# ipfs/go-libp2p-pubsub

Measured on AMD Instinct MI355X. Metric: deliveries/sec (peer×msg) at 1M peers, 1/2/4/8 GPU; % of HBM roofline, higher is better.
Workload: dtype u64

## Files before the change

### go-libp2p-pubsub_amd/csrc/api.cpp

```cpp
#include <algorithm>
#include <cstdio>
#include <cstdlib>
#include <cstring>

#include "engine.hpp"
#include "psengine_plan.h"

using namespace psamd;

namespace {

TopicHost* join_topic(ps_engine* e, uint32_t topic) {
  if (!topic_ok(e, topic)) {
    e->fail(PS_E_STATE, "no such topic");
    return nullptr;
  }
  TopicHost& T = e->topics[topic];
  if (T.kind != Kind::Join) {
    e->fail(PS_E_STATE, "topic topology was set explicitly");
    return nullptr;
  }
  return &T;
}

// ... 117 lines not shown
  d.timing = env_flag("PSAMD_DRAIN_TIMING", d.timing);
  if (!env_flag("PSAMD_AB", false)) return;
  d.slab_ids = std::max<uint64_t>(kDrainSegBits, env_u64("PSAMD_DRAIN_SLAB_IDS", 10, d.slab_ids));
  if (const char* v = std::getenv("PSAMD_DRAIN_EMIT")) d.staged = std::strcmp(v, "direct") != 0;
  if (const char* v = std::getenv("PSAMD_DRAIN_ASYNC_OUT")) d.mapped_out = std::strcmp(v, "mapped") == 0;
  if (const char* v = std::getenv("PSAMD_DRAIN_SHARED")) d.share = std::strcmp(v, "private") != 0;
  if (const char* v = std::getenv("PSAMD_LOAD_COUNT")) d.load_rows = std::strcmp(v, "rows") == 0;
  d.spread_wide = env_u32("PSAMD_SPREAD_WIDE", 0, 1 << 30, d.spread_wide);
  d.spread_track_levels = env_u32("PSAMD_SPREAD_TRACK_LEVELS", 0, kAny, d.spread_track_levels);
  s.twin = env_flag("PSAMD_TWIN", s.twin);
  s.expand_opts = env_flag("PSAMD_NARROW", true) ? 0u : kExpandNoNarrow;
  s.chain_words_lead = env_u32("PSAMD_CHAIN_WORDS_LEAD", 0, 1 << 20, s.chain_words_lead);
  s.upload_reuse = env_flag("PSAMD_UPLOAD_REUSE", s.upload_reuse);
  s.sig_windows = env_flag("PSAMD_SIG_WINDOWS", s.sig_windows);
  s.fuse_reduce = env_flag("PSAMD_FUSE_REDUCE", s.fuse_reduce);
  ps_plan_opts o = e->opts;
  o.gpu_build = env_flag("PSAMD_GPU_BUILD", o.gpu_build);
  o.flood = env_flag("PSAMD_FLOOD", o.flood);
  if (!env_flag("PSAMD_PULL_PAIR", true)) o.chain_max = o.chain_max_groups = 1;
  if (const char* v = std::getenv("PSAMD_XCHG_OVERLAP")) o.xchg_overlap = std::atoi(v) != 0;
  o.chain_max = env_u32("PSAMD_CHAIN", 1, kChainLevels, o.chain_max);
  o.chain_max_groups = env_u32("PSAMD_CHAIN", 1, kChainLevels, o.chain_max_groups);
  o.overlap = env_flag("PSAMD_OVERLAP", o.overlap);
  o.overlap_min_rounds = env_u32("PSAMD_OVERLAP_ROUNDS", 2, kAny, o.overlap_min_rounds);
  o.overlap_min_bytes = env_u64("PSAMD_OVERLAP_BYTES", 10, o.overlap_min_bytes);
  o.pad_words = env_u32("PSAMD_PAD_WORDS", 2, kAny, o.pad_words);
  o.chain_tail = env_flag("PSAMD_CHAIN_TAIL", o.chain_tail);
  if (const char* v = std::getenv("PSAMD_LAUNCH_BYTES"))
    o.launch_bytes = static_cast<uint64_t>(std::max(0.0, std::atof(v)));
  o.chain_words = env_u32("PSAMD_CHAIN_WORDS", 256, 1 << 20, o.chain_words);
// ... 446 lines not shown
      got.emplace_back((static_cast<uint64_t>(e->last_msgs[i].start) << 32) | i, e->last_first + i);
  }
  std::sort(got.begin(), got.end());
  *n_out = got.size();
  if (got.size() > cap) return e->fail(PS_E_RANGE, "output buffer too small");
  for (size_t k = 0; k < got.size(); ++k) msg_out[k] = got[k].second;
  return PS_OK;
}

int ps_overlapped_windows(ps_engine* e, uint64_t* count_out) {
  if (!e || !count_out) return PS_E_INVAL;
  *count_out = e->overlapped;
  return PS_OK;
}

int ps_seen_digest(ps_engine* e, uint64_t* digest_out) {
  if (!e || !digest_out) return PS_E_INVAL;
  if (!e->have_window) return e->fail(PS_E_NOTREADY, "no completed run");
  if (const int rj = twin_join(e)) return rj;
  HIP_TRY(hipMemsetAsync(e->d_digest.p, 0, 8, e->stream), "clear digest");
  const bool timed = e->drain.env.timing && e->drain.ev_t[0];
  if (timed) HIP_TRY(hipEventRecord(e->drain.ev_t[0], e->stream), "event");
  HIP_TRY(launch_digest(e->rows.seen.as<uint64_t>(), e->rows.gen.as<uint8_t>(), e->rows.gen_cur, e->d_node_peer.as<uint32_t>(),
                        e->d_node_topic.as<uint16_t>(),
                        e->last_slot->topics.as<TopicDev>(), e->last_slot->groups.as<GroupDev>(), e->n_nodes, e->d_digest.as<uint64_t>(), e->stream),
          "digest");
  if (timed) HIP_TRY(hipEventRecord(e->drain.ev_t[1], e->stream), "event");
  HIP_TRY(hipMemcpyAsync(digest_out, e->d_digest.p, 8, hipMemcpyDeviceToHost, e->stream), "read digest");
  HIP_TRY(hipStreamSynchronize(e->stream), "sync");
  if (timed) {
// ... 300 lines not shown
    case PS_PLAN_CHAIN: {
      const PairPlan& P = e->pair;
      if (index >= P.len.size() || P.len[index] < 3) {
        v = {0};
        break;
      }
      v = {P.len[index]};
      for (uint32_t k = P.lo[index]; k < P.hi[index]; ++k) {
        const ChainChunk& c = P.chain[k];
        v.insert(v.end(), {c.node_begin, c.node_end, c.topic, c.W, static_cast<uint64_t>(c.row0_hi) << 32 | c.row0_lo,
                           c.w0, c.S, c.levels, c.r0, c.group});
        for (uint32_t f = 0; f <= kChainLevels; ++f) v.push_back(c.first[f]);
      }
      break;
    }
    case PS_PLAN_SCHEDULE: {
      if (!L) return e->fail(PS_E_RANGE, "no window planned");
      const WindowSchedule& S = e->probe_sched;
      const size_t lv = L->level ? 1 : 0;
      v = {S.flood_rounds, S.pre_P, S.n_slots, S.reach_rows, S.mode, S.total, lv * S.lgrid.size(),
           lv * e->woff_host.size(), lv * e->desc_host.size(), S.seed_off.size()};
      if (lv) {
        v.insert(v.end(), S.lgrid.begin(), S.lgrid.end());
        v.insert(v.end(), e->woff_host.begin(), e->woff_host.end());
        v.insert(v.end(), e->desc_host.begin(), e->desc_host.end());
      }
      v.insert(v.end(), S.seed_off.begin(), S.seed_off.end());
      break;
    }
    default:
// ... 69 lines not shown
```

### go-libp2p-pubsub_amd/csrc/engine.hpp

```cpp
#pragma once
#include <hip/hip_runtime.h>

#include <array>
#include <chrono>
#include <cstdlib>
#include <cstdint>
#include <map>
#include <memory>
#include <string>
#include <utility>
#include <vector>

#include "dist.hpp"
#include "kernels.hpp"
#include "psengine.h"
#include "tree.hpp"

namespace psamd {

constexpr uint32_t kMaxRoundsCap = 4096;
constexpr uint32_t kAlignedRowsMax = 2 * (PS_MAX_ROUNDS + 1);
constexpr uint32_t kMaxStartRound = 200;
constexpr uint32_t kDefaultWindow = 65536;
constexpr uint32_t kMaxWindow = 1u << 30;
// ... 141 lines not shown
struct PullPlan {
  std::vector<uint64_t> key;
  uint64_t version = 0;
  std::vector<PullChunk> chunks;
  std::vector<uint32_t> off, gsplit;
  std::vector<uint64_t> bytes;
};
struct PairPlan {
  std::vector<uint64_t> key;
  uint64_t version = 0;
  std::vector<PullChunk> chunks;
  std::vector<ChainChunk> chain;
  std::vector<uint32_t> lo, hi, gsplit;
  std::vector<uint32_t> len;
  std::vector<uint8_t> kind;
};
struct FloodPlan {
  std::vector<uint64_t> key;
  uint64_t version = 0;
  std::vector<FloodTask> tasks;
  std::vector<FloodSeg> segs;
  std::vector<uint32_t> slot0, nslot;
  uint32_t slots = 1;
  uint32_t granules = 0;
};
struct GhostRound {
  std::vector<uint64_t> s_off, s_len, r_off, r_len;
  uint32_t pack0 = 0, pack1 = 0;
  uint64_t pack_units = 0;
  bool any = false;
// ... 42 lines not shown
  hipStream_t xstream = nullptr;
  hipEvent_t ev_run0 = nullptr, ev_run1 = nullptr;
  hipEvent_t ev_round = nullptr, ev_xchg = nullptr;
  ps_plan_opts opts = psamd::default_plan_opts();
  bool xchg_overlap = true;
  struct Switches {
    bool host_timing = false;
    bool flood_profile = false;
    std::string chain_prof_path;
    bool twin = true;
    bool sig_windows = true;
    bool fuse_reduce = true;
    bool upload_reuse = true;
    uint32_t expand_opts = 0;
    uint32_t chain_words_lead = 0;
  } env;
  std::vector<hipEvent_t> ev_k;
  uint32_t n_cus = 256, expand_grid = 2048;
  bool host_only = false;
  psamd::WindowLayout probe;
  psamd::WindowSchedule probe_sched;
  struct UploadShadow {
    uint64_t gen = 0;
    std::vector<uint8_t> data;
  };
  std::map<const psamd::DevBuf*, UploadShadow> upload_shadow;
  bool defer_into_signalled = false;
  uint64_t sig_seq = 0;
  struct PendingReduce {
    bool valid = false;
// ... 41 lines not shown
  bool graph_dirty = true, flags_dirty = true;
  uint64_t graph_epoch = 0, flags_epoch = 0;

  std::vector<uint32_t> woff_host, desc_host;
  psamd::DevBuf d_reach;
  std::vector<psamd::ReachPiece> reach_host;
  std::vector<uint64_t> reach_key;
  uint32_t n_reach = 0, reach_a = 0;
  psamd::PullPlan pull;
  psamd::DevBuf d_pull;
  uint64_t pull_up = ~0ull;
  psamd::DevBuf d_chain;
  std::vector<uint64_t> chain_fail_key;
  psamd::DevBuf d_chain_ovf;
  psamd::DevBuf d_chain_meta, d_chain_cnt, d_chain_scan;
  static constexpr uint64_t kNtBytes = 64ull << 20;
  psamd::PairPlan pair;
  psamd::DevBuf d_pp;
  uint64_t pair_up = ~0ull;
  std::vector<uint8_t> round_kind;

  uint32_t n_nodes = 0, n_pad = 16;
  std::vector<uint32_t> node_peer, row_ptr, col;
  std::vector<uint32_t> node_parent;
  std::vector<uint16_t> node_topic;
  std::vector<uint8_t> node_flags;

  psamd::DevBuf d_row_ptr, d_col, d_node_topic, d_node_flags, d_node_peer, d_node_parent;
  psamd::DevBuf d_ext0, d_ext1;
  struct RowSet {
// ... 368 lines not shown
    uint64_t epoch = ~0ull;
    std::vector<uint32_t> gslot;
    std::vector<uint32_t> plist;
    std::vector<std::vector<uint32_t>> pl_off;
    psamd::DevBuf d_gslot, d_plist;
  } dist_slots;

  struct Staging {
    uint8_t* h = nullptr;
    uint8_t* d = nullptr;
    size_t cap = 0;
  };
  struct RunSlot {
    Staging stg;
    psamd::DevBuf topics, woff, groups, partials, seeds;
    hipEvent_t ev_gate = nullptr;
    ps_stats st{};
    bool deferred = false;
    uint32_t r = 0, launches = 0;
    uint32_t mode = PS_MODE_COMPACT, flood_rounds = 0;
    hipEvent_t ev0 = nullptr, ev1 = nullptr;
    uint64_t* hs = nullptr;
    uint64_t* hs_dev = nullptr;
    uint64_t* ha = nullptr;
    uint64_t* sig = nullptr;
    uint64_t* sig_dev = nullptr;
    uint64_t seq = 0;
    bool signalled = false;
    uint32_t planned0 = 0;
    uint32_t true_rounds = 0;
// ... 119 lines not shown
```

### go-libp2p-pubsub_amd/csrc/kernels.hpp

```cpp
#pragma once
#include <hip/hip_runtime.h>

#include <cstdint>

namespace psamd {

enum : uint8_t {
  kNodeLive = 1,
  kNodeInternal = 2,
  kNodeSplit = 4,
};

constexpr uint32_t kRemoteBit = 0x80000000u;
constexpr uint32_t kRemoteRankShift = 27;
constexpr uint32_t kRemoteIdMask = (1u << kRemoteRankShift) - 1u;
constexpr int kMaxRanks = 16;

struct XItem {
  uint32_t node;
  uint32_t word;
  uint64_t mask;
};
constexpr uint32_t kRegionHeader = 16;

// ... 165 lines not shown
  uint32_t first[kChainLevels + 1];
  uint32_t lo[kChainLevels], hi[kChainLevels];
  uint32_t nbase, root;
};
static_assert(sizeof(ChainChunk) == 128, "two chunk descriptors per 256-B line");
hipError_t launch_chain_ranges(ChainChunk* chunks, uint32_t n, const uint32_t* row_ptr, uint32_t cap,
                               uint32_t* overflow, hipStream_t s);
hipError_t launch_chain_meta(ChainChunk* chunks, uint32_t n, const uint32_t* node_parent, const uint8_t* node_flags,
                             uint32_t* counts, void* scan_temp, size_t scan_bytes, uint32_t* meta, bool fill,
                             hipStream_t s);
size_t chain_meta_scan_bytes(uint32_t n);
hipError_t launch_pull_chain(const PullArgs& a, const ChainChunk* chunks, uint32_t n_chunks, uint32_t round,
                             bool record, bool nt, bool slices, bool inner_nt, uint32_t waves_per_cu,
                             hipStream_t s);
hipError_t launch_chain_parents(ChainChunk* chunks, uint32_t n, const uint32_t* node_parent, hipStream_t s);
constexpr uint32_t kPullSlots = 256;
constexpr uint32_t kPairSlots = kPullSlots;

struct FloodTask {
  uint32_t nb, ne;
  uint32_t topic, round;
  uint32_t slot0, nslot;
  uint32_t g_own, gsz;
  uint32_t p_lo, p_hi;
  uint32_t pg_lo, pg_hi;
  uint32_t pnode0, pgsz;
  uint32_t pseg;
  uint32_t seg;
};
struct FloodSeg {
// ... 727 lines not shown
```

### go-libp2p-pubsub_amd/csrc/plan.cpp

```cpp
#include <algorithm>
#include <cstring>

#include "engine.hpp"

namespace psamd {

uint64_t phys_word(const TopicDev& d, const std::vector<StartGroup>& G, uint64_t u, uint32_t w) {
  if (!(d.flags & kTopicGroups)) return d.wbase + u * d.W + w;
  for (const StartGroup& g : G)
    if (w < g.w0 + g.wn) return d.wbase + static_cast<uint64_t>(d.n_nodes) * g.w0 + u * g.wn + (w - g.w0);
  return d.wbase;
}

namespace {

uint32_t block_w(const TopicDev& d, const StartGroup& g) { return (d.flags & kTopicGroups) ? g.wn : d.W; }
uint64_t block_row0(const TopicDev& d, const StartGroup& g) {
  return d.wbase + ((d.flags & kTopicGroups) ? static_cast<uint64_t>(d.n_nodes) * g.w0 : 0);
}

}

int plan_window_layout(ps_engine* e, const std::vector<RunMsg>& msgs, const std::vector<WinSlice>& win,
                       WindowLayout& L) {
// ... 343 lines not shown
      if (!can(q, len)) continue;
      const double c = wb + rd[q] + (wb > 0 ? kLaunchBytes : 0.0) + best[q + len];
      if (c < best[q]) {
        best[q] = c;
        take[q] = static_cast<uint8_t>(len);
      }
    }
  }
  auto& C = PP.chunks;
  C.clear();
  PP.chain.clear();
  PP.lo.assign(rounds + 2, 0);
  PP.hi.assign(rounds + 2, 0);
  PP.gsplit.assign(rounds + 2, 0);
  PP.len.assign(rounds + 2, 0);
  const bool gpu = e->gpu_graph;
  std::vector<PullChunk> ghost;
  for (uint32_t q = first + 1; q <= rounds; ++q) {
    const uint32_t len = take[q];
    if (len == 1) {
      kind[q] = e->pull.bytes[q] ? PS_K_PULL : PS_K_NONE;
      continue;
    }
    PP.len[q] = len;
    if (len >= 3) {
      kind[q] = PS_K_CHAIN;
      for (uint32_t k = 1; k < len; ++k) kind[q + k] = PS_K_CHAIN2;
      PP.lo[q] = static_cast<uint32_t>(PP.chain.size());
      std::vector<ChainChunk> sliced;
      chain_parts(q, len, [&](uint32_t t, uint32_t gi, uint32_t d, uint32_t r0, uint32_t levels) {
// ... 17 lines not shown
            c.w0 = w0;
            c.S = std::min(z.S, W - w0);
            c.levels = static_cast<uint8_t>(levels);
            c.r0 = static_cast<uint8_t>(r0);
            c.group = static_cast<uint16_t>(gi);
            c.nbase = T.nbase;
            c.root = T.root_local ? T.nbase : kNoneNode;
            for (uint32_t k = 0; k <= levels && k <= kChainLevels; ++k)
              c.first[k] = T.nbase + (d + k < T.level_off.size() ? T.level_off[d + k] : T.n_nodes);
            (z.S < W ? sliced : PP.chain).push_back(c);
          }
      });
      PP.gsplit[q] = static_cast<uint32_t>(PP.chain.size());
      PP.chain.insert(PP.chain.end(), sliced.begin(), sliced.end());
      PP.hi[q] = static_cast<uint32_t>(PP.chain.size());
      q += len - 1;
      continue;
    }
    kind[q] = PS_K_PAIR;
    kind[q + 1] = PS_K_PAIR2;
    PP.lo[q] = static_cast<uint32_t>(C.size());
    ghost.clear();
    for (uint32_t t = 0; t < nt; ++t) {
      const TopicHost& T = e->topics[t];
      if (tab[t].W == 0) continue;
      for (uint32_t gi = 0; gi < L.groups[t].size(); ++gi) {
        const StartGroup& g = L.groups[t][gi];
        const uint32_t W = block_w(tab[t], g);
        uint32_t d, per;
        bool late = false;
// ... 570 lines not shown
```

### go-libp2p-pubsub_amd/csrc/run.cpp

```cpp
#include <algorithm>
#include <chrono>
#include <atomic>
#include <cstdio>
#include <cstdlib>
#include <cstring>
#include <iterator>
#include <thread>

#include "engine.hpp"
#include "gbuild.hpp"

namespace {
inline void cpu_relax() {
#if defined(__x86_64__) || defined(__i386__)
  __builtin_ia32_pause();
#else
  std::this_thread::yield();
#endif
}
}

namespace psamd {

namespace {
// ... 53 lines not shown
    uint32_t back[2] = {0, 0};
    HIP_TRY(hipMemcpyAsync(&back[0], e->d_chain_ovf.p, 4, hipMemcpyDeviceToHost, e->stream), "read chain overflow");
    HIP_TRY(hipMemcpyAsync(&back[1], e->d_chain_cnt.as<uint32_t>() + nk + 1 + nk, 4, hipMemcpyDeviceToHost,
                           e->stream),
            "read chain entries");
    HIP_TRY(hipStreamSynchronize(e->stream), "sync");
    if (back[0]) {
      *overflow = true;
      return PS_OK;
    }
    HIP_TRY(e->d_chain_meta.ensure(std::max<size_t>(back[1], 1) * 4), "alloc chain entries");
    HIP_TRY(launch_chain_meta(e->d_chain.as<ChainChunk>(), nk, e->d_node_parent.as<uint32_t>(),
                              e->d_node_flags.as<uint8_t>(), e->d_chain_cnt.as<uint32_t>(), nullptr, 0,
                              e->d_chain_meta.as<uint32_t>(), true, e->stream),
            "chain entries");
  }
  e->pair_up = e->pair.version;
  return PS_OK;
}

int upload_flood(ps_engine* e) {
  if (e->flood.version == e->flood_up) return PS_OK;
  const auto& TK = e->flood.tasks;
  const auto& SG = e->flood.segs;
  const size_t n = TK.size();
  HIP_TRY(e->d_flood_tasks.ensure(std::max<size_t>(n, 1) * sizeof(FloodTask)), "alloc flood tasks");
  HIP_TRY(e->d_flood_segs.ensure(std::max<size_t>(SG.size(), 1) * sizeof(FloodSeg)), "alloc flood segments");
  bool fresh = false;
  HIP_TRY(e->d_flood_gran.ensure(std::max<size_t>(e->flood.granules, 1) * 8, &fresh), "alloc flood granules");
  if (fresh) HIP_TRY(hipMemsetAsync(e->d_flood_gran.p, 0, e->d_flood_gran.bytes, e->stream), "clear granules");
// ... 198 lines not shown
  uint32_t reach_a = 0;
  bool twin = false, pcap = false, alt_sets = false, overlap = false, fold = false, sigwin = false;
  std::vector<uint64_t> gkey;
  WindowStart ws{};
  const void* staged[4] = {nullptr, nullptr, nullptr, nullptr};
  ExpandArgs a{};
  PullArgs pa{};
  uint64_t* arr[2] = {nullptr, nullptr};
  uint64_t* partials = nullptr;
  uint64_t* stats = nullptr;
  uint32_t stats_rows = 0, n_waves = 0;
  bool upfront = false;
  bool zero_copy = false;
  std::vector<const uint8_t*> peer_region;
  bool gate_done = false, reach_a_done = false;
  bool cprof = false;
  bool host_stats_written = false;
  bool reduce_side = false;
  size_t ev_used = 0;
  std::vector<uint32_t> ev_round;
  uint32_t launches = 0;
  uint32_t r = 0;
  std::vector<uint64_t> s_off, s_len, r_off, r_len;
  Clock::time_point t_w0, t_w1, t_w3, t_first, t_enq;

  bool defers(uint32_t r) {
    return e->defer_last && e->defer_into && !record && !timed && r <= PS_MAX_ROUNDS &&
           (e->world == 1 || L.planned0 <= PS_MAX_ROUNDS);
  }

// ... 450 lines not shown
  }

  int launch_chain(uint32_t r, bool xr) {
    const uint32_t len = e->pair.len[r];
    const uint32_t last = r + len - 1;
    const bool ntc =
        last == L.planned0 || (last < e->pull.bytes.size() && e->pull.bytes[last] >= ps_engine::kNtBytes);
    pa.slot_mod = kPairSlots;
    pa.row_ptr = e->d_row_ptr.as<uint32_t>();
    for (uint32_t k = 0; k < kChainLevels; ++k)
      pa.partials_r[k] = k < len ? partials + static_cast<size_t>(e->woff_host[r + k]) * kNumCtr : nullptr;
    HIP_TRY(time_mark(true), "event");
    ++launches;
    uint64_t* const prof = cprof ? e->d_chain_prof.as<uint64_t>() : nullptr;
    pa.prof = prof ? prof + static_cast<size_t>(e->pair.lo[r]) * kChainProf : nullptr;
    HIP_TRY(launch_pull_chain(pa, e->d_chain.as<ChainChunk>() + e->pair.lo[r], e->pair.gsplit[r] - e->pair.lo[r], r,
                              record, ntc, false, e->opts.chain_nt, e->opts.chain_waves, s),
            "pull chain");
    pa.prof = prof ? prof + static_cast<size_t>(e->pair.gsplit[r]) * kChainProf : nullptr;
    HIP_TRY(launch_pull_chain(pa, e->d_chain.as<ChainChunk>() + e->pair.gsplit[r], e->pair.hi[r] - e->pair.gsplit[r],
                              r, record, ntc, true, e->opts.chain_nt, e->opts.chain_waves, s),
            "pull chain (column slices)");
    pa.prof = nullptr;
    HIP_TRY(time_mark(false), "event");
    if (xr) HIP_TRY(hipStreamWaitEvent(s, e->ev_xchg, 0), "exchange join");
    return PS_OK;
  }

  int launch_pull_round(uint32_t r, bool pair, bool xr, hipStream_t xs) {
    const uint32_t rw = pair ? r + 1 : r;
    const bool nt = rw < e->pull.bytes.size() && (e->pull.bytes[rw] >= ps_engine::kNtBytes || rw == L.planned0);
    pa.partials = partials + static_cast<size_t>(e->woff_host[r]) * kNumCtr;
    pa.slot_mod = pair ? kPairSlots : kPullSlots;
// ... 781 lines not shown
```

### go-libp2p-pubsub_amd/psengine/__init__.py

```python
from __future__ import annotations

import ctypes as C
import os

import numpy as np

from . import _build

NONE = 0xFFFFFFFF
HOP_NONE = 0xFF
MAX_ROUNDS = 256

PS_OK = 0
ERRORS = {
    -1: "PS_E_INVAL", -2: "PS_E_NOMEM", -3: "PS_E_STATE", -4: "PS_E_NOPARENT",
    -5: "PS_E_UNREACHABLE", -6: "PS_E_DEVICE", -7: "PS_E_RANGE", -8: "PS_E_NOTREADY",
}
PART_PEER = 0
PART_SUBTREE = 1
F_RECORD_HOPS = 0x1
F_TIME_KERNELS = 0x2
F_NO_LAZY_SEEN = 0x4
F_COMPACT = 0x8
MODE_COMPACT, MODE_LEVEL_PULL, MODE_FLOOD = 0, 2, 3
# ... 162 lines not shown
    ("ps_blame_track", C.c_int, [_P, _u32p, C.c_size_t, C.c_size_t]),
    ("ps_blame_take", C.c_int, [_P, C.POINTER(_u64p), C.POINTER(_u32p), C.POINTER(_u32p), C.POINTER(_u32p),
                                C.POINTER(_u32p), C.POINTER(_u32p), _u64p, _u64p, _u64p, _u64p]),
    ("ps_peer_report", C.c_int, [_P, _u32p, C.c_size_t, C.c_uint32, C.POINTER(Report), C.c_size_t]),
    ("ps_report_track", C.c_int, [_P, _u32p, C.c_size_t, C.c_uint32]),
    ("ps_report_take", C.c_int, [_P, C.POINTER(Report), C.c_size_t, _u64p, _u64p]),
    ("ps_dist_report", C.c_int, [_P, _u32p, C.c_size_t, C.c_uint32, C.POINTER(Report), C.c_size_t]),
    ("ps_dist_cut", C.c_int, [_P, _u32p, C.c_size_t, _u64p, _u64p, _u64p, _u64p]),
    ("ps_dist_blame", C.c_int, [_P, _u32p, C.c_size_t, C.POINTER(_u64p), C.POINTER(_u32p), C.POINTER(_u32p),
                                C.POINTER(_u32p), C.POINTER(_u32p), C.POINTER(_u32p), _u64p]),
    ("ps_topic_spread", C.c_int, [_P, _u32p, C.c_size_t, _u64p, _u64p, _u64p, _u64p, _u64p, _u64p]),
    ("ps_spread_track", C.c_int, [_P, _u32p, C.c_size_t]),
    ("ps_spread_take", C.c_int, [_P, _u64p, _u64p, _u64p, _u64p, _u64p, _u64p, _u64p, _u64p]),
    ("ps_seen_digest", C.c_int, [_P, _u64p]),
    ("ps_overlapped_windows", C.c_int, [_P, _u64p]),
    ("ps_msg_encode", C.c_int, [C.POINTER(MessageC), C.c_char_p, C.c_size_t, C.POINTER(C.c_size_t)]),
    ("ps_msg_decode", C.c_int, [C.c_char_p, C.c_size_t, C.POINTER(MessageBuf), C.POINTER(C.c_size_t)]),
    ("ps_dist_unique_id", C.c_int, [C.POINTER(C.c_uint8)]),
    ("ps_dist_init", C.c_int, [_P, C.POINTER(DistConfig), C.POINTER(C.c_uint8)]),
    ("ps_device_count", C.c_int, [_i32p]),
    ("ps_dist_ipc_id", C.c_int, [C.POINTER(C.c_uint8)]),
    ("ps_dist_init_ipc", C.c_int, [_P, C.POINTER(DistConfig), C.POINTER(C.c_uint8)]),
    ("ps_loopback_create", C.c_int, [C.c_int32, C.POINTER(_P)]),
    ("ps_loopback_destroy", None, [_P]),
    ("ps_dist_init_loopback", C.c_int, [_P, C.POINTER(DistConfig), _P]),
    ("ps_partition_owner", C.c_int, [_u32, _u32, _u32p, _u32, C.POINTER(DistConfig), _i32p]),
]

G_NODE_PEER, G_NODE_PARENT, G_NODE_TOPIC, G_NODE_FLAGS, G_ROW_PTR, G_COL, G_TOPIC, G_BUILD = range(8)
NODE_LIVE, NODE_INTERNAL, NODE_SPLIT = 1, 2, 4
# ... 669 lines not shown
        from . import plan

        return graph_get(plan.lib(), self._h, what, index)

    def graph_topic(self, topic: int) -> dict:
        return graph_topic(self.graph(G_TOPIC, topic))

    def build_report(self) -> dict:
        return build_report(self.graph(G_BUILD))

    def overlapped_windows(self) -> int:
        d = C.c_uint64()
        self._check(self._L.ps_overlapped_windows(self._h, C.byref(d)))
        return d.value

    def dist_init(self, rank: int, world: int, unique_id: bytes, partition: int = PART_PEER,
                  split_depth: int = 0):
        dc = DistConfig(rank, world, partition, split_depth)
        uid = (C.c_uint8 * 128).from_buffer_copy(unique_id)
        self._check(self._L.ps_dist_init(self._h, C.byref(dc), uid))

    def dist_init_ipc(self, rank: int, world: int, group_id: bytes, partition: int = PART_PEER,
                      split_depth: int = 0, copy: bool = False, inplace: bool = False):
        flags = (DIST_F_COPY if copy else 0) | (DIST_F_INPLACE if inplace else 0)
        dc = DistConfig(rank, world, partition, split_depth, flags, 0)
        gid = (C.c_uint8 * 128).from_buffer_copy(group_id)
        self._check(self._L.ps_dist_init_ipc(self._h, C.byref(dc), gid))

    def dist_init_loopback(self, group: "Loopback", rank: int, partition: int = PART_PEER,
                           split_depth: int = 0, copy: bool = False, inplace: bool = False):
# ... 69 lines not shown
```

### go-libp2p-pubsub_amd/psengine/_build.py

```python
from __future__ import annotations

import os
import subprocess

PKG = os.path.dirname(os.path.dirname(os.path.abspath(__file__)))
REPO = os.path.dirname(PKG)
CSRC = os.path.join(PKG, "csrc")
LIBDIR = os.path.join(PKG, "lib")
LIB = os.path.join(LIBDIR, "libpsengine.so")
HIPCC = os.environ.get("HIPCC", "/opt/rocm/bin/hipcc")
ARCH = "gfx950"

SOURCES = ["kernels.hip", "pull.hip", "flood.hip", "gbuild.hip", "drain.hip", "graph.cpp", "plan.cpp", "run.cpp", "api.cpp",
           "drain_tables.cpp", "drain_standing.cpp", "drain.cpp", "drain_shared.cpp", "drain_sink.cpp", "drain_topics.cpp",
           "drain_load.cpp", "drain_hops.cpp", "drain_downstream.cpp", "drain_cut.cpp", "drain_report.cpp",
           "drain_dist.cpp", "drain_spread.cpp", "drain_blame.cpp", "drain_blame_track.cpp", "drain_spread_track.cpp",
           "tree.cpp", "dist.cpp", "codec.cpp", "pubsub.cpp"]
HEADERS = ["kernels.hpp", "devutil.hpp", "gbuild.hpp", "tree.hpp", "dist.hpp", "engine.hpp", "drain_impl.hpp"]


def _stale() -> bool:
    if not os.path.exists(LIB):
        return True
    t = os.path.getmtime(LIB)
    deps = [os.path.join(CSRC, f) for f in SOURCES + HEADERS]
    deps.append(os.path.join(REPO, "include", "psengine.h"))
    deps.append(os.path.join(REPO, "include", "pubsub.hpp"))
    deps.append(os.path.join(REPO, "include", "psengine_plan.h"))
# ... 56 lines not shown
```

### go-libp2p-pubsub_amd/psengine/plan.py

```python
from __future__ import annotations

import ctypes as C

import numpy as np

from . import (DistConfig, EngineError, G_BUILD, G_TOPIC, PART_PEER, PlanOpts, _P, _p, _u32arr, build_report,
               graph_get, graph_topic, load)

(INFO, NODES, PARENT, GHOST_REF, TOPIC, LAYOUT, ROUND_KIND, PULL, PAIR, XCHG, SEGS, SHIP, PACK, CHAIN,
 SCHEDULE) = range(15)
CHAIN_FIELDS = ("node_begin", "node_end", "topic", "W", "row0", "w0", "S", "levels", "r0", "group")
CHAIN_LEVELS = 6
CHUNK_FIELDS = ("node_begin", "node_end", "topic", "W", "row0", "e_lo", "e_hi", "gin", "gout", "group",
                "p_lo", "p_hi", "c_lo")
PROTOTYPES = [
    ("ps_plan_create", C.c_int, [C.c_uint32, C.c_uint32, C.POINTER(C.c_uint32), C.POINTER(C.c_uint32),
                                 C.POINTER(DistConfig), C.POINTER(_P)]),
    ("ps_plan_destroy", None, [_P]),
    ("ps_plan_set_msg_window", C.c_int, [_P, C.c_uint32]),
    ("ps_plan_window", C.c_int, [_P, C.POINTER(C.c_uint32), C.POINTER(C.c_uint32), C.c_size_t, C.c_uint32]),
    ("ps_plan_get", C.c_int, [_P, C.c_uint32, C.c_uint32, C.POINTER(C.c_uint64), C.c_size_t,
                              C.POINTER(C.c_size_t)]),
    ("ps_graph_get", C.c_int, [_P, C.c_uint32, C.c_uint32, C.POINTER(C.c_uint64), C.c_size_t,
                               C.POINTER(C.c_size_t)]),
]
# ... 142 lines not shown
        out["desc"] = out["desc"].reshape(-1, 3)
        return out

    def chain(self, q: int):
        v = self.get(CHAIN, q)
        n = int(v[0])
        if n == 0:
            return 0, []
        body = v[1:].reshape(-1, len(CHAIN_FIELDS) + CHAIN_LEVELS + 1)
        out = []
        for row in body:
            c = dict(zip(CHAIN_FIELDS, (int(x) for x in row[:len(CHAIN_FIELDS)])))
            c["first"] = [int(x) for x in row[len(CHAIN_FIELDS):]]
            out.append(c)
        return n, out
```

### include/psengine.h

```cpp
#ifndef PSENGINE_H
#define PSENGINE_H

#include <stddef.h>
#include <stdint.h>

#ifdef __cplusplus
extern "C" {
#endif

#define PS_NONE 0xFFFFFFFFu
#define PS_HOP_NONE 0xFFu
#define PS_MAX_ROUNDS 256

enum ps_status {
  PS_OK = 0,
  PS_E_INVAL = -1,
  PS_E_NOMEM = -2,
  PS_E_STATE = -3,
  PS_E_NOPARENT = -4,
  PS_E_UNREACHABLE = -5,
  PS_E_DEVICE = -6,
  PS_E_RANGE = -7,
  PS_E_NOTREADY = -8
};
// ... 264 lines not shown

int ps_topic_spread(ps_engine* e, const uint32_t* topic, size_t n,
                    uint64_t* reached_out, uint64_t* deliv_out,
                    uint64_t* unreached_out, uint64_t* stranded_out,
                    uint64_t* copies_out, uint64_t* dup_out);
int ps_spread_track(ps_engine* e, const uint32_t* topic, size_t n);
int ps_spread_take(ps_engine* e,
                   uint64_t* reached_out, uint64_t* deliv_out,
                   uint64_t* unreached_out, uint64_t* stranded_out,
                   uint64_t* copies_out, uint64_t* dup_out,
                   uint64_t* n_windows_out, uint64_t* n_truncated_out);
int ps_seen_digest(ps_engine* e, uint64_t* digest_out);

int ps_overlapped_windows(ps_engine* e, uint64_t* count_out);

#define PS_PART_PEER 0u
#define PS_PART_SUBTREE 1u
#define PS_UNIQUE_ID_BYTES 128

typedef struct ps_dist_config {
  int32_t rank;
  int32_t world;
  uint32_t partition;
  uint32_t split_depth;
  uint32_t flags;
  uint32_t reserved;
} ps_dist_config;
#define PS_DIST_F_COPY 0x1u
#define PS_DIST_F_INPLACE 0x2u

// ... 52 lines not shown
```

### include/psengine_plan.h

```cpp
#ifndef PSENGINE_PLAN_H
#define PSENGINE_PLAN_H

#include "psengine.h"

#ifdef __cplusplus
extern "C" {
#endif

int ps_plan_create(uint32_t n_peers, uint32_t n_topics, const uint32_t* roots, const uint32_t* parents,
                   const ps_dist_config* dc, ps_engine** out);
void ps_plan_destroy(ps_engine* e);
int ps_plan_set_msg_window(ps_engine* e, uint32_t msg_window);
int ps_plan_window(ps_engine* e, const uint32_t* topic_of_msg, const uint32_t* start_round, size_t n_msgs,
                   uint32_t flags);

#define PS_PLAN_INFO 0
#define PS_PLAN_NODES 1
#define PS_PLAN_PARENT 2
#define PS_PLAN_GHOST_REF 3
#define PS_PLAN_TOPIC 4
#define PS_PLAN_LAYOUT 5
#define PS_PLAN_ROUND_KIND 6
#define PS_PLAN_PULL 7
#define PS_PLAN_PAIR 8
#define PS_PLAN_XCHG 9
#define PS_PLAN_SEGS 10
#define PS_PLAN_SHIP 11
#define PS_PLAN_PACK 12
#define PS_PLAN_CHAIN 13
#define PS_PLAN_SCHEDULE 14
int ps_plan_get(ps_engine* e, uint32_t what, uint32_t index, uint64_t* out, size_t cap, size_t* n_out);

#define PS_GRAPH_NODE_PEER 0
#define PS_GRAPH_NODE_PARENT 1
#define PS_GRAPH_NODE_TOPIC 2
#define PS_GRAPH_NODE_FLAGS 3
#define PS_GRAPH_ROW_PTR 4
#define PS_GRAPH_COL 5
#define PS_GRAPH_TOPIC 6
#define PS_GRAPH_BUILD 7
int ps_graph_get(ps_engine* e, uint32_t what, uint32_t index, uint64_t* out, size_t cap, size_t* n_out);

#ifdef __cplusplus
}
#endif
// ... 2 lines not shown
```

Baseline: 40030 billion.

## Replace chain pull with split reach and row-fill kernels for single-GPU windows

```diff
diff --git a/go-libp2p-pubsub_amd/csrc/api.cpp b/go-libp2p-pubsub_amd/csrc/api.cpp
--- a/go-libp2p-pubsub_amd/csrc/api.cpp
+++ b/go-libp2p-pubsub_amd/csrc/api.cpp
@@ -155,6 +155,11 @@
   s.upload_reuse = env_flag("PSAMD_UPLOAD_REUSE", s.upload_reuse);
   s.sig_windows = env_flag("PSAMD_SIG_WINDOWS", s.sig_windows);
   s.fuse_reduce = env_flag("PSAMD_FUSE_REDUCE", s.fuse_reduce);
+  s.chain_fill = env_flag("PSAMD_CHAIN_FILL", s.chain_fill);
+  s.chain_fill_bytes = env_u64("PSAMD_CHAIN_FILL_BYTES", 10, s.chain_fill_bytes);
+  s.chain_fill_row_words = env_u64("PSAMD_CHAIN_FILL_ROW_WORDS", 10, s.chain_fill_row_words);
+  s.chain_fill_waves = env_u32("PSAMD_CHAIN_FILL_WAVES", 0, 32, s.chain_fill_waves);
+  s.chain_fill_piece = env_u32("PSAMD_CHAIN_FILL_PIECE", 16, 1 << 16, s.chain_fill_piece);
   ps_plan_opts o = e->opts;
   o.gpu_build = env_flag("PSAMD_GPU_BUILD", o.gpu_build);
   o.flood = env_flag("PSAMD_FLOOD", o.flood);
@@ -631,6 +636,12 @@
   return PS_OK;
 }
 
+int ps_chain_fill_launches(ps_engine* e, uint64_t* count_out) {
+  if (!e || !count_out) return PS_E_INVAL;
+  *count_out = e->chain_fills;
+  return PS_OK;
+}
+
 int ps_seen_digest(ps_engine* e, uint64_t* digest_out) {
   if (!e || !digest_out) return PS_E_INVAL;
   if (!e->have_window) return e->fail(PS_E_NOTREADY, "no completed run");
@@ -961,6 +972,27 @@
       }
       break;
     }
+    case PS_PLAN_FILL: {
+      const PairPlan& P = e->pair;
+      if (index >= P.fill_hi.size() || P.fill_hi[index] <= P.fill_lo[index]) {
+        v = {0};
+        break;
+      }
+      v = {P.fill_hi[index] - P.fill_lo[index], P.fill_np[index], P.fill_blocks[index]};
+      for (uint32_t k = P.fill_lo[index]; k < P.fill_hi[index]; ++k) {
+        const FillSeg& f = P.fill[k];
+        v.insert(v.end(), {f.topic, f.W, f.row0, f.nbase, f.levels, f.piece0, f.blk0, f.pw});
+        for (uint32_t i = 0; i <= kChainLevels; ++i) v.push_back(f.first[i]);
+      }
+      for (uint32_t k = P.fill_lo[index]; k < P.fill_hi[index]; ++k) {
+        const FillSeg& f = P.fill[k];
+        for (uint32_t j = 0, n = fill_seg_pieces(f); j < n; ++j) {
+          const FillPiece p = fill_piece(f, j);
+          v.insert(v.end(), {p.w0, p.nw, p.node0, p.off0});
+        }
+      }
+      break;
+    }
     case PS_PLAN_SCHEDULE: {
       if (!L) return e->fail(PS_E_RANGE, "no window planned");
       const WindowSchedule& S = e->probe_sched;
diff --git a/go-libp2p-pubsub_amd/csrc/engine.hpp b/go-libp2p-pubsub_amd/csrc/engine.hpp
--- a/go-libp2p-pubsub_amd/csrc/engine.hpp
+++ b/go-libp2p-pubsub_amd/csrc/engine.hpp
@@ -179,6 +179,8 @@
   std::vector<uint32_t> lo, hi, gsplit;
   std::vector<uint32_t> len;
   std::vector<uint8_t> kind;
+  std::vector<FillSeg> fill;
+  std::vector<uint32_t> fill_lo, fill_hi, fill_blocks, fill_p0, fill_np;
 };
 struct FloodPlan {
   std::vector<uint64_t> key;
@@ -251,6 +253,11 @@
     bool upload_reuse = true;
     uint32_t expand_opts = 0;
     uint32_t chain_words_lead = 0;
+    bool chain_fill = true;
+    uint32_t chain_fill_piece = psamd::kFillPieceWords;
+    uint64_t chain_fill_bytes = 512ull << 20;
+    uint64_t chain_fill_row_words = psamd::kFillMinRowWords;
+    uint32_t chain_fill_waves = psamd::kFillWaves;
   } env;
   std::vector<hipEvent_t> ev_k;
   uint32_t n_cus = 256, expand_grid = 2048;
@@ -322,6 +329,8 @@
   std::vector<uint64_t> chain_fail_key;
   psamd::DevBuf d_chain_ovf;
   psamd::DevBuf d_chain_meta, d_chain_cnt, d_chain_scan;
+  psamd::DevBuf d_fill_segs, d_fill_pieces;
+  uint64_t chain_fills = 0;
   static constexpr uint64_t kNtBytes = 64ull << 20;
   psamd::PairPlan pair;
   psamd::DevBuf d_pp;
@@ -720,6 +729,7 @@
   struct RunSlot {
     Staging stg;
     psamd::DevBuf topics, woff, groups, partials, seeds;
+    psamd::DevBuf fill_pop;
     hipEvent_t ev_gate = nullptr;
     ps_stats st{};
     bool deferred = false;
diff --git a/go-libp2p-pubsub_amd/csrc/fill.hip b/go-libp2p-pubsub_amd/csrc/fill.hip
--- /dev/null
+++ b/go-libp2p-pubsub_amd/csrc/fill.hip
@@ -0,0 +1,219 @@
+#include <cstddef>
+
+#include "devutil.hpp"
+#include "kernels.hpp"
+
+namespace psamd {
+
+namespace {
+
+using namespace dev;
+
+typedef unsigned int u32x4 __attribute__((ext_vector_type(4)));
+
+__global__ __launch_bounds__(kBlock) void k_fill_pieces(const FillSeg* __restrict__ segs, uint32_t n_segs,
+                                                        FillPiece* __restrict__ pieces, uint32_t n_pieces) {
+  const uint32_t i = blockIdx.x * kBlock + threadIdx.x;
+  if (i >= n_pieces) return;
+  uint32_t lo = 0, hi = n_segs;
+  while (hi - lo > 1) {
+    const uint32_t mid = (lo + hi) >> 1;
+    if (segs[mid].piece0 <= i)
+      lo = mid;
+    else
+      hi = mid;
+  }
+  pieces[i] = fill_piece(segs[lo], i - segs[lo].piece0);
+}
+
+__global__ __launch_bounds__(64) void k_fill_popc(const FillSeg* __restrict__ segs, uint32_t n_segs,
+                                                  const uint64_t* __restrict__ a_cur, uint32_t* __restrict__ pop) {
+  const uint32_t si = blockIdx.x;
+  if (si >= n_segs) return;
+  const uint64_t* row = a_cur + segs[si].row0;
+  const uint32_t W = segs[si].W;
+  uint32_t n = 0;
+  for (uint32_t i = threadIdx.x; i < W; i += 64) n += static_cast<uint32_t>(__popcll(row[i]));
+  n = __reduce_add_sync(~0ull, n);
+  if (threadIdx.x == 0) pop[segs[si].topic] = n;
+}
+
+__device__ __forceinline__ uint64_t* fill_slots(const FillReachArgs& a, uint32_t i) {
+  switch (i) {
+    case 0: return a.partials_r[0];
+    case 1: return a.partials_r[1];
+    case 2: return a.partials_r[2];
+    case 3: return a.partials_r[3];
+    case 4: return a.partials_r[4];
+    default: return a.partials_r[5];
+  }
+}
+
+__global__ __launch_bounds__(kFillReachBlock) void k_fill_reach(FillReachArgs a) {
+  const uint32_t b = blockIdx.x;
+  uint32_t lo = 0, hi = a.n_segs;
+  while (hi - lo > 1) {
+    const uint32_t mid = (lo + hi) >> 1;
+    if (a.segs[mid].blk0 <= b)
+      lo = mid;
+    else
+      hi = mid;
+  }
+  const FillSeg* const S = a.segs + lo;
+  const uint32_t levels = S->levels, W = S->W, cur = a.gen_cur & 0xFF;
+  const uint32_t u0 = S->first[0], end = S->first[levels];
+  const uint32_t u = u0 + (b - S->blk0) * kFillReachBlock + threadIdx.x;
+  const bool in = u < end;
+  const uint32_t uc = in ? u : u0;
+  uint32_t k = 0;
+  for (uint32_t j = 1; j < kChainLevels; ++j) k += (j < levels && uc >= S->first[j]) ? 1u : 0u;
+  const uint32_t par = a.node_parent[uc];
+  const uint32_t par_prev = a.node_parent[uc - 1];
+  const bool live = a.node_flags[uc] & kNodeLive;
+  uint32_t p = par;
+  bool live_above = true;
+  for (uint32_t j = 0; j < k; ++j) {
+    live_above = live_above && (a.node_flags[p] & kNodeLive);
+    p = a.node_parent[p];
+  }
+  const bool up = in && live_above && a.gen[p] == cur;
+  const bool ok = up && live;
+  const bool first = up && par != par_prev;
+  if (ok) a.gen[uc] = static_cast<uint8_t>(cur);
+  const uint32_t lane = threadIdx.x & 63u, wave = threadIdx.x >> 6;
+  const uint64_t slot = (static_cast<uint64_t>(b) * (kFillReachBlock / 64) + wave) % a.slot_mod;
+  const uint64_t pop = a.pop[S->topic];
+  for (uint32_t j = 0; j < levels; ++j) {
+    const uint64_t nodes = __ballot(in && k == j);
+    if (nodes == 0) continue;
+    const uint64_t reached = __popcll(__ballot(ok && k == j));
+    const uint64_t parents = __popcll(__ballot(first && k == j));
+    const uint64_t pwords = (j == 0 && b == S->blk0 && wave == 0) ? W : 0u;
+    const uint64_t v7[7] = {reached * pop, reached * W, static_cast<uint64_t>(__popcll(nodes)), reached, parents,
+                            pwords, 0ull};
+    uint64_t* const partials = fill_slots(a, j);
+    if (partials && lane < kNumCtr) {
+      const uint64_t v = pull_ctr_pick(v7, lane);
+      if (v) atomicAdd(reinterpret_cast<unsigned long long*>(partials + slot * kNumCtr + lane),
+                       static_cast<unsigned long long>(v));
+    }
+  }
+}
+
+template <bool kNT>
+__device__ __forceinline__ void fill_store16(uint64_t* p, const u32x4& v) {
+  if constexpr (kNT)
+    __builtin_nontemporal_store(v, reinterpret_cast<u32x4*>(p));
+  else
+    *reinterpret_cast<u32x4*>(p) = v;
+}
+
+template <bool kNT>
+__global__ __launch_bounds__(64) void k_fill_rows(const FillPiece* __restrict__ pieces, uint32_t n_pieces,
+                                                  const uint64_t* __restrict__ a_cur, uint64_t* __restrict__ seen,
+                                                  const uint8_t* __restrict__ gen, uint32_t gen_cur) {
+  constexpr uint32_t kU = 8;
+  constexpr uint32_t kGenWords = (kFillPieceNodes + 2 + 3) / 4 + 2;
+  __shared__ __attribute__((aligned(16))) uint64_t row[kChainWords];
+  __shared__ uint32_t genl[kGenWords];
+  if (blockIdx.x >= n_pieces) return;
+  const FillPiece* const pc = pieces + blockIdx.x;
+  const uint32_t lane = threadIdx.x;
+  const uint32_t cur = gen_cur & 0xFF;
+  const uint64_t w0 = pc->w0;
+  const uint32_t nw = pc->nw, W = pc->W, node0 = pc->node0, off0 = pc->off0;
+  const uint64_t* const src = a_cur + pc->row0;
+  const uint32_t nn = (off0 + nw + W - 1) / W;
+  const uint32_t g0 = node0 & ~3u;
+  const uint32_t nd = (((node0 + nn + 3u) & ~3u) - g0) >> 2;
+  const uint32_t* const gen32 = reinterpret_cast<const uint32_t*>(gen + g0);
+  for (uint32_t i = lane; i < nd; i += 64) genl[i] = gen32[i];
+  for (uint32_t i = lane; i < W; i += 64) row[i] = src[i];
+  __syncthreads();
+  const uint8_t* const genb = reinterpret_cast<const uint8_t*>(genl) + (node0 - g0);
+  const float rw = 1.0f / static_cast<float>(W);
+  auto split = [&](uint32_t i, int32_t& kk, int32_t& r) {
+    const uint32_t li = off0 + i;
+    kk = static_cast<int32_t>(static_cast<float>(li) * rw);
+    r = static_cast<int32_t>(li) - kk * static_cast<int32_t>(W);
+    const int32_t lo = r < 0, hi = r >= static_cast<int32_t>(W);
+    kk += hi - lo;
+    r += (lo - hi) * static_cast<int32_t>(W);
+  };
+  auto word = [&](uint32_t i) {
+    int32_t kk, r;
+    split(i, kk, r);
+    return genb[kk] == cur ? row[r] : 0ull;
+  };
+  uint64_t* const out = seen + w0;
+  const uint32_t h = static_cast<uint32_t>(w0 & 1u);
+  const uint32_t nu = (nw - h) >> 1;
+  if (h && lane == 0) out[0] = word(0);
+  if (((nw - h) & 1u) && lane == 1) out[nw - 1] = word(nw - 1);
+  const bool even = !(W & 1u) && !((off0 + h) & 1u);
+  for (uint32_t c0 = 0; c0 < nu; c0 += kU * 64) {
+    u32x4 x[kU];
+#pragma unroll
+    for (uint32_t q = 0; q < kU; ++q) {
+      const uint32_t c = min(c0 + q * 64 + lane, nu - 1);
+      int32_t kk, r;
+      split(h + 2 * c, kk, r);
+      if (even) {
+        x[q] = genb[kk] == cur ? *reinterpret_cast<const u32x4*>(row + r) : u32x4{0, 0, 0, 0};
+      } else {
+        const uint64_t a0 = genb[kk] == cur ? row[r] : 0ull;
+        const bool wrap = static_cast<uint32_t>(r) + 1 == W;
+        const uint64_t a1 = genb[kk + (wrap ? 1 : 0)] == cur ? row[wrap ? 0 : r + 1] : 0ull;
+        x[q] = u32x4{static_cast<uint32_t>(a0), static_cast<uint32_t>(a0 >> 32), static_cast<uint32_t>(a1),
+                     static_cast<uint32_t>(a1 >> 32)};
+      }
+    }
+#pragma unroll
+    for (uint32_t q = 0; q < kU; ++q) {
+      const uint32_t c = c0 + q * 64 + lane;
+      if (c < nu) fill_store16<kNT>(out + h + 2 * c, x[q]);
+    }
+  }
+}
+
+}
+
+hipError_t launch_fill_pieces(const FillSeg* segs, uint32_t n_segs, FillPiece* pieces, uint32_t n_pieces,
+                              hipStream_t s) {
+  if (n_segs == 0 || n_pieces == 0) return hipSuccess;
+  hipLaunchKernelGGL(k_fill_pieces, dim3((n_pieces + kBlock - 1) / kBlock), dim3(kBlock), 0, s, segs, n_segs, pieces,
+                     n_pieces);
+  return hipGetLastError();
+}
+
+hipError_t launch_fill_popc(const FillSeg* segs, uint32_t n_segs, const uint64_t* a_cur, uint32_t* pop, hipStream_t s) {
+  if (n_segs == 0) return hipSuccess;
+  hipLaunchKernelGGL(k_fill_popc, dim3(n_segs), dim3(64), 0, s, segs, n_segs, a_cur, pop);
+  return hipGetLastError();
+}
+
+hipError_t launch_fill_reach(const FillReachArgs& a, uint32_t n_blocks, hipStream_t s) {
+  if (a.n_segs == 0 || n_blocks == 0) return hipSuccess;
+  hipLaunchKernelGGL(k_fill_reach, dim3(n_blocks), dim3(kFillReachBlock), 0, s, a);
+  return hipGetLastError();
+}
+
+hipError_t launch_fill_rows(const FillPiece* pieces, uint32_t n_pieces, const uint64_t* a_cur, uint64_t* seen,
+                            const uint8_t* gen, uint32_t gen_cur, uint32_t waves_per_cu, hipStream_t s) {
+  if (n_pieces == 0) return hipSuccess;
+  static const size_t fixed = [] {
+    hipFuncAttributes fa{};
+    return hipFuncGetAttributes(&fa, reinterpret_cast<const void*>(k_fill_rows<false>)) == hipSuccess
+               ? fa.sharedSizeBytes
+               : size_t{0};
+  }();
+  size_t pad = 0;
+  if (waves_per_cu) {
+    const size_t per = (160u * 1024u) / waves_per_cu - 512u;
+    pad = per > fixed ? per - fixed : 0;
+  }
+  hipLaunchKernelGGL(k_fill_rows<false>, dim3(n_pieces), dim3(64), pad, s, pieces, n_pieces, a_cur, seen, gen, gen_cur);
+  return hipGetLastError();
+}
+
+}
diff --git a/go-libp2p-pubsub_amd/csrc/kernels.hpp b/go-libp2p-pubsub_amd/csrc/kernels.hpp
--- a/go-libp2p-pubsub_amd/csrc/kernels.hpp
+++ b/go-libp2p-pubsub_amd/csrc/kernels.hpp
@@ -203,6 +203,77 @@
                              bool record, bool nt, bool slices, bool inner_nt, uint32_t waves_per_cu,
                              hipStream_t s);
 hipError_t launch_chain_parents(ChainChunk* chunks, uint32_t n, const uint32_t* node_parent, hipStream_t s);
+struct FillSeg {
+  uint64_t row0;
+  uint32_t topic, W;
+  uint32_t nbase, levels;
+  uint32_t first[kChainLevels + 1];
+  uint32_t piece0;
+  uint32_t blk0;
+  uint32_t pw;
+};
+static_assert(sizeof(FillSeg) == 64, "four segments per 256-B line");
+struct FillPiece {
+  uint64_t w0, row0;
+  uint32_t nw, W;
+  uint32_t node0, off0;
+};
+static_assert(sizeof(FillPiece) == 32, "one scalar load per wave");
+constexpr uint32_t kFillLine = 16;
+constexpr uint32_t kFillPieceWords = 2048;
+constexpr uint32_t kFillPieceNodes = 2048;
+constexpr uint32_t kFillWaves = 16;
+constexpr uint32_t kFillReachBlock = 256;
+constexpr uint32_t kFillMinRowWords = 128;
+__host__ __device__ inline uint64_t fill_seg_begin(const FillSeg& s) {
+  return s.row0 + static_cast<uint64_t>(s.first[0] - s.nbase) * s.W;
+}
+__host__ __device__ inline uint64_t fill_seg_end(const FillSeg& s) {
+  return s.row0 + static_cast<uint64_t>(s.first[s.levels] - s.nbase) * s.W;
+}
+__host__ __device__ inline uint32_t fill_piece_words(uint32_t W, uint32_t words) {
+  const uint64_t cap = (static_cast<uint64_t>(kFillPieceNodes) * W) & ~static_cast<uint64_t>(kFillLine - 1);
+  const uint32_t w = (words < kFillLine ? kFillLine : words) & ~(kFillLine - 1);
+  return cap < w ? static_cast<uint32_t>(cap < kFillLine ? kFillLine : cap) : w;
+}
+__host__ __device__ inline uint32_t fill_seg_pieces(const FillSeg& s) {
+  const uint64_t wb = fill_seg_begin(s), we = fill_seg_end(s);
+  if (we <= wb) return 0;
+  const uint64_t a = wb & ~static_cast<uint64_t>(kFillLine - 1);
+  return static_cast<uint32_t>((we - a + s.pw - 1) / s.pw);
+}
+__host__ __device__ inline FillPiece fill_piece(const FillSeg& s, uint32_t j) {
+  const uint64_t wb = fill_seg_begin(s), we = fill_seg_end(s);
+  const uint64_t a = wb & ~static_cast<uint64_t>(kFillLine - 1);
+  const uint64_t b = a + static_cast<uint64_t>(j) * s.pw, e = b + s.pw;
+  FillPiece p;
+  p.w0 = b < wb ? wb : b;
+  p.row0 = s.row0;
+  p.nw = static_cast<uint32_t>((e > we ? we : e) - p.w0);
+  p.W = s.W;
+  const uint64_t rel = p.w0 - s.row0;
+  p.node0 = s.nbase + static_cast<uint32_t>(rel / s.W);
+  p.off0 = static_cast<uint32_t>(rel % s.W);
+  return p;
+}
+struct FillReachArgs {
+  const FillSeg* segs;
+  uint32_t n_segs;
+  const uint32_t* node_parent;
+  const uint8_t* node_flags;
+  uint8_t* gen;
+  uint32_t gen_cur;
+  const uint32_t* pop;
+  uint64_t* partials_r[kChainLevels];
+  uint32_t slot_mod;
+};
+hipError_t launch_fill_pieces(const FillSeg* segs, uint32_t n_segs, FillPiece* pieces, uint32_t n_pieces,
+                              hipStream_t s);
+hipError_t launch_fill_popc(const FillSeg* segs, uint32_t n_segs, const uint64_t* a_cur, uint32_t* pop, hipStream_t s);
+hipError_t launch_fill_reach(const FillReachArgs& a, uint32_t n_blocks, hipStream_t s);
+hipError_t launch_fill_rows(const FillPiece* pieces, uint32_t n_pieces, const uint64_t* a_cur, uint64_t* seen,
+                            const uint8_t* gen, uint32_t gen_cur, uint32_t waves_per_cu, hipStream_t s);
+
 constexpr uint32_t kPullSlots = 256;
 constexpr uint32_t kPairSlots = kPullSlots;
 
diff --git a/go-libp2p-pubsub_amd/csrc/plan.cpp b/go-libp2p-pubsub_amd/csrc/plan.cpp
--- a/go-libp2p-pubsub_amd/csrc/plan.cpp
+++ b/go-libp2p-pubsub_amd/csrc/plan.cpp
@@ -381,6 +381,10 @@
   PP.hi.assign(rounds + 2, 0);
   PP.gsplit.assign(rounds + 2, 0);
   PP.len.assign(rounds + 2, 0);
+  PP.fill.clear();
+  for (auto* v : {&PP.fill_lo, &PP.fill_hi, &PP.fill_blocks, &PP.fill_p0, &PP.fill_np}) v->assign(rounds + 2, 0);
+  uint32_t fill_pieces = 0;
+  const bool fill_ok = e->env.chain_fill && e->world == 1 && !L.multi && !L.aligned && L.max_start == 0;
   const bool gpu = e->gpu_graph;
   std::vector<PullChunk> ghost;
   for (uint32_t q = first + 1; q <= rounds; ++q) {
@@ -428,6 +432,48 @@
       PP.gsplit[q] = static_cast<uint32_t>(PP.chain.size());
       PP.chain.insert(PP.chain.end(), sliced.begin(), sliced.end());
       PP.hi[q] = static_cast<uint32_t>(PP.chain.size());
+      if (fill_ok) {
+        const uint32_t s0 = static_cast<uint32_t>(PP.fill.size());
+        uint64_t words = 0, launch_nodes = 0;
+        uint32_t blocks = 0, pieces = 0;
+        bool ok = true;
+        chain_parts(q, len, [&](uint32_t t, uint32_t gi, uint32_t d, uint32_t r0, uint32_t levels) {
+          const TopicHost& T = e->topics[t];
+          const StartGroup& g = L.groups[t][gi];
+          const uint32_t W = block_w(tab[t], g);
+          if (chain_size(T, d, levels, W, words_of(q, len)).S < W) return;
+          ok = ok && r0 == 0 && g.start == 0 && d >= 1 && T.root_local && !(tab[t].flags & kTopicGroups);
+          FillSeg f{};
+          f.row0 = block_row0(tab[t], g);
+          f.topic = t;
+          f.W = W;
+          f.nbase = T.nbase;
+          f.levels = levels;
+          f.pw = fill_piece_words(W, e->env.chain_fill_piece);
+          for (uint32_t k = 0; k <= levels && k <= kChainLevels; ++k)
+            f.first[k] = T.nbase + (d + k < T.level_off.size() ? T.level_off[d + k] : T.n_nodes);
+          const uint32_t nodes = f.first[levels] - f.first[0];
+          if (nodes == 0) return;
+          f.piece0 = pieces;
+          f.blk0 = blocks;
+          pieces += fill_seg_pieces(f);
+          blocks += (nodes + kFillReachBlock - 1) / kFillReachBlock;
+          words += static_cast<uint64_t>(nodes) * W;
+          launch_nodes += nodes;
+          PP.fill.push_back(f);
+        });
+        if (ok && words * 8 >= e->env.chain_fill_bytes && words >= e->env.chain_fill_row_words * launch_nodes &&
+            PP.fill.size() > s0) {
+          PP.fill_lo[q] = s0;
+          PP.fill_hi[q] = static_cast<uint32_t>(PP.fill.size());
+          PP.fill_blocks[q] = blocks;
+          PP.fill_p0[q] = fill_pieces;
+          PP.fill_np[q] = pieces;
+          fill_pieces += pieces;
+        } else {
+          PP.fill.resize(s0);
+        }
+      }
       q += len - 1;
       continue;
     }
diff --git a/go-libp2p-pubsub_amd/csrc/run.cpp b/go-libp2p-pubsub_amd/csrc/run.cpp
--- a/go-libp2p-pubsub_amd/csrc/run.cpp
+++ b/go-libp2p-pubsub_amd/csrc/run.cpp
@@ -91,6 +91,22 @@
                               e->d_node_flags.as<uint8_t>(), e->d_chain_cnt.as<uint32_t>(), nullptr, 0,
                               e->d_chain_meta.as<uint32_t>(), true, e->stream),
             "chain entries");
+    const auto& F = e->pair.fill;
+    if (!F.empty()) {
+      uint32_t np = 0;
+      for (size_t q = 0; q < e->pair.fill_np.size(); ++q) np += e->pair.fill_np[q];
+      HIP_TRY(e->d_fill_segs.ensure(F.size() * sizeof(FillSeg)), "alloc fill segments");
+      HIP_TRY(e->d_fill_pieces.ensure(std::max<size_t>(np, 1) * sizeof(FillPiece)), "alloc fill pieces");
+      HIP_TRY(hipMemcpyAsync(e->d_fill_segs.p, F.data(), F.size() * sizeof(FillSeg), hipMemcpyHostToDevice, e->stream),
+              "upload fill segments");
+      for (size_t q = 0; q < e->pair.fill_np.size(); ++q)
+        if (e->pair.fill_hi[q] > e->pair.fill_lo[q])
+          HIP_TRY(launch_fill_pieces(e->d_fill_segs.as<FillSeg>() + e->pair.fill_lo[q],
+                                     e->pair.fill_hi[q] - e->pair.fill_lo[q],
+                                     e->d_fill_pieces.as<FillPiece>() + e->pair.fill_p0[q], e->pair.fill_np[q],
+                                     e->stream),
+                  "fill pieces");
+    }
   }
   e->pair_up = e->pair.version;
   return PS_OK;
@@ -319,6 +335,7 @@
   bool zero_copy = false;
   std::vector<const uint8_t*> peer_region;
   bool gate_done = false, reach_a_done = false;
+  bool fill_pop_done = false;
   bool cprof = false;
   bool host_stats_written = false;
   bool reduce_side = false;
@@ -799,9 +816,36 @@
     ++launches;
     uint64_t* const prof = cprof ? e->d_chain_prof.as<uint64_t>() : nullptr;
     pa.prof = prof ? prof + static_cast<size_t>(e->pair.lo[r]) * kChainProf : nullptr;
-    HIP_TRY(launch_pull_chain(pa, e->d_chain.as<ChainChunk>() + e->pair.lo[r], e->pair.gsplit[r] - e->pair.lo[r], r,
-                              record, ntc, false, e->opts.chain_nt, e->opts.chain_waves, s),
-            "pull chain");
+    const uint32_t f0 = e->pair.fill_lo[r], f1 = e->pair.fill_hi[r];
+    const bool fill = f1 > f0 && !record && !cprof && !pa.all_current && e->world == 1 && upfront && !xr &&
+                      (!pcap || alt_sets);
+    if (fill) {
+      const FillSeg* const segs = e->d_fill_segs.as<FillSeg>() + f0;
+      if (!fill_pop_done) {
+        HIP_TRY(slot->fill_pop.ensure(std::max<size_t>(nt, 1) * 4), "alloc root row counts");
+        HIP_TRY(launch_fill_popc(segs, f1 - f0, pa.a_cur, slot->fill_pop.as<uint32_t>(), s), "root row counts");
+        fill_pop_done = true;
+      }
+      FillReachArgs fa{};
+      fa.segs = segs;
+      fa.n_segs = f1 - f0;
+      fa.node_parent = pa.node_parent;
+      fa.node_flags = pa.node_flags;
+      fa.gen = pa.gen;
+      fa.gen_cur = pa.gen_cur;
+      fa.pop = slot->fill_pop.as<uint32_t>();
+      for (uint32_t k = 0; k < kChainLevels; ++k) fa.partials_r[k] = pa.partials_r[k];
+      fa.slot_mod = e->woff_host[r + 1] - e->woff_host[r];
+      HIP_TRY(launch_fill_reach(fa, e->pair.fill_blocks[r], s), "fill reach");
+      HIP_TRY(launch_fill_rows(e->d_fill_pieces.as<FillPiece>() + e->pair.fill_p0[r], e->pair.fill_np[r], pa.a_cur,
+                               pa.seen, pa.gen, pa.gen_cur, e->env.chain_fill_waves, s),
+              "fill rows");
+      ++e->chain_fills;
+    } else {
+      HIP_TRY(launch_pull_chain(pa, e->d_chain.as<ChainChunk>() + e->pair.lo[r], e->pair.gsplit[r] - e->pair.lo[r], r,
+                                record, ntc, false, e->opts.chain_nt, e->opts.chain_waves, s),
+              "pull chain");
+    }
     pa.prof = prof ? prof + static_cast<size_t>(e->pair.gsplit[r]) * kChainProf : nullptr;
     HIP_TRY(launch_pull_chain(pa, e->d_chain.as<ChainChunk>() + e->pair.gsplit[r], e->pair.hi[r] - e->pair.gsplit[r],
                               r, record, ntc, true, e->opts.chain_nt, e->opts.chain_waves, s),
diff --git a/go-libp2p-pubsub_amd/psengine/__init__.py b/go-libp2p-pubsub_amd/psengine/__init__.py
--- a/go-libp2p-pubsub_amd/psengine/__init__.py
+++ b/go-libp2p-pubsub_amd/psengine/__init__.py
@@ -200,6 +200,7 @@
     ("ps_spread_take", C.c_int, [_P, _u64p, _u64p, _u64p, _u64p, _u64p, _u64p, _u64p, _u64p]),
     ("ps_seen_digest", C.c_int, [_P, _u64p]),
     ("ps_overlapped_windows", C.c_int, [_P, _u64p]),
+    ("ps_chain_fill_launches", C.c_int, [_P, _u64p]),
     ("ps_msg_encode", C.c_int, [C.POINTER(MessageC), C.c_char_p, C.c_size_t, C.POINTER(C.c_size_t)]),
     ("ps_msg_decode", C.c_int, [C.c_char_p, C.c_size_t, C.POINTER(MessageBuf), C.POINTER(C.c_size_t)]),
     ("ps_dist_unique_id", C.c_int, [C.POINTER(C.c_uint8)]),
@@ -899,6 +900,11 @@
         self._check(self._L.ps_overlapped_windows(self._h, C.byref(d)))
         return d.value
 
+    def chain_fill_launches(self) -> int:
+        d = C.c_uint64()
+        self._check(self._L.ps_chain_fill_launches(self._h, C.byref(d)))
+        return d.value
+
     def dist_init(self, rank: int, world: int, unique_id: bytes, partition: int = PART_PEER,
                   split_depth: int = 0):
         dc = DistConfig(rank, world, partition, split_depth)
diff --git a/go-libp2p-pubsub_amd/psengine/_build.py b/go-libp2p-pubsub_amd/psengine/_build.py
--- a/go-libp2p-pubsub_amd/psengine/_build.py
+++ b/go-libp2p-pubsub_amd/psengine/_build.py
@@ -11,7 +11,7 @@
 HIPCC = os.environ.get("HIPCC", "/opt/rocm/bin/hipcc")
 ARCH = "gfx950"
 
-SOURCES = ["kernels.hip", "pull.hip", "flood.hip", "gbuild.hip", "drain.hip", "graph.cpp", "plan.cpp", "run.cpp", "api.cpp",
+SOURCES = ["kernels.hip", "pull.hip", "fill.hip", "flood.hip", "gbuild.hip", "drain.hip", "graph.cpp", "plan.cpp", "run.cpp", "api.cpp",
            "drain_tables.cpp", "drain_standing.cpp", "drain.cpp", "drain_shared.cpp", "drain_sink.cpp", "drain_topics.cpp",
            "drain_load.cpp", "drain_hops.cpp", "drain_downstream.cpp", "drain_cut.cpp", "drain_report.cpp",
            "drain_dist.cpp", "drain_spread.cpp", "drain_blame.cpp", "drain_blame_track.cpp", "drain_spread_track.cpp",
diff --git a/go-libp2p-pubsub_amd/psengine/plan.py b/go-libp2p-pubsub_amd/psengine/plan.py
--- a/go-libp2p-pubsub_amd/psengine/plan.py
+++ b/go-libp2p-pubsub_amd/psengine/plan.py
@@ -8,7 +8,9 @@
                graph_get, graph_topic, load)
 
 (INFO, NODES, PARENT, GHOST_REF, TOPIC, LAYOUT, ROUND_KIND, PULL, PAIR, XCHG, SEGS, SHIP, PACK, CHAIN,
- SCHEDULE) = range(15)
+ SCHEDULE, FILL) = range(16)
+FILL_FIELDS = ("topic", "W", "row0", "nbase", "levels", "piece0", "blk0", "pw")
+FILL_PIECE_FIELDS = ("w0", "nw", "node0", "off0")
 CHAIN_FIELDS = ("node_begin", "node_end", "topic", "W", "row0", "w0", "S", "levels", "r0", "group")
 CHAIN_LEVELS = 6
 CHUNK_FIELDS = ("node_begin", "node_end", "topic", "W", "row0", "e_lo", "e_hi", "gin", "gout", "group",
@@ -181,3 +183,19 @@
             c["first"] = [int(x) for x in row[len(CHAIN_FIELDS):]]
             out.append(c)
         return n, out
+
+    def fill(self, q: int):
+        v = self.get(FILL, q).astype(np.int64)
+        ns = int(v[0])
+        if ns == 0:
+            return 0, [], []
+        n_pieces, blocks = int(v[1]), int(v[2])
+        per = len(FILL_FIELDS) + CHAIN_LEVELS + 1
+        segs = []
+        for row in v[3:3 + ns * per].reshape(ns, per):
+            f = dict(zip(FILL_FIELDS, (int(x) for x in row[:len(FILL_FIELDS)])))
+            f["first"] = [int(x) for x in row[len(FILL_FIELDS):]]
+            segs.append(f)
+        body = v[3 + ns * per:].reshape(n_pieces, len(FILL_PIECE_FIELDS))
+        pieces = [dict(zip(FILL_PIECE_FIELDS, (int(x) for x in row))) for row in body]
+        return blocks, segs, pieces
diff --git a/include/psengine.h b/include/psengine.h
--- a/include/psengine.h
+++ b/include/psengine.h
@@ -302,6 +302,8 @@
 
 int ps_overlapped_windows(ps_engine* e, uint64_t* count_out);
 
+int ps_chain_fill_launches(ps_engine* e, uint64_t* count_out);
+
 #define PS_PART_PEER 0u
 #define PS_PART_SUBTREE 1u
 #define PS_UNIQUE_ID_BYTES 128
diff --git a/include/psengine_plan.h b/include/psengine_plan.h
--- a/include/psengine_plan.h
+++ b/include/psengine_plan.h
@@ -29,6 +29,7 @@
 #define PS_PLAN_PACK 12
 #define PS_PLAN_CHAIN 13
 #define PS_PLAN_SCHEDULE 14
+#define PS_PLAN_FILL 15
 int ps_plan_get(ps_engine* e, uint32_t what, uint32_t index, uint64_t* out, size_t cap, size_t* n_out);
 
 #define PS_GRAPH_NODE_PEER 0
```

Result: faster. 43170 billion, median of 6 (+7.8%).
